# lasgroup/safe-adaptation-gym

Hardware: NVIDIA B200
Metric: env_steps_per_sec_point_go_to_goal (higher is better)
Workload: dtype f64

## Files before the change

include/sag_b200.h:

```cpp
#ifndef SAG_B200_H
#define SAG_B200_H
#include <stddef.h>
#include <stdint.h>

#ifdef __cplusplus
extern "C" {
#endif

#define SAG_ABI_VERSION 3
#define SAG_LIDAR_BINS 16
#define SAG_OBS_POINT 60
#define SAG_OBS_CAR 72
#define SAG_MAX_SLOTS 32
#define SAG_MAX_GREMLINS 4

enum { SAG_ROBOT_POINT = 0, SAG_ROBOT_CAR = 1 };
enum {
  SAG_T_CATCH_GOAL = 0, SAG_T_COLLECT, SAG_T_DRIBBLE_BALL, SAG_T_GO_TO_GOAL, SAG_T_GO_TO_GOAL_DAMPING,
  SAG_T_GO_TO_GOAL_MOTOR, SAG_T_GO_TO_GOAL_SCARCE, SAG_T_HAUL_BOX, SAG_T_PRESS_BUTTONS,
  SAG_T_PRESS_BUTTONS_SCARCE, SAG_T_PUSH_BOX, SAG_T_PUSH_BOX_SCARCE, SAG_T_ROLL_ROD, SAG_T_UNSUPERVISED,
  SAG_NUM_TASKS
};
enum { SAG_FLAG_PHYSICS_ERROR = 1, SAG_FLAG_RESAMPLE_FAILED = 2, SAG_FLAG_NEEDS_RESET = 4 };
enum { SAG_ERR_BAD_TASK_ID = 8 };

typedef struct SagConfig {
  int32_t n_envs;
  int32_t robot;
  uint64_t seed;
  uint32_t env_id_base;
  int32_t max_episode_steps;
  int32_t max_layout_draws;
  int32_t random_bound;
  double placements_margin, robot_keepout;
  double hazards_size, vases_size, pillars_size, gremlins_size;
  double hazards_keepout, gremlins_keepout, vases_keepout, pillars_keepout;
  double gremlins_travel, robot_ctrl_range_scale, action_noise, max_bound;
  int32_t num_gremlins;
  int32_t reserved_;
} SagConfig;

enum {
  SAG_F_ROBOT = 0,
  SAG_F_OBJECTS = 1,
  SAG_F_TASK_F64 = 2,
  SAG_F_TASK_I32 = 3,
  SAG_F_FLAGS = 4,
  SAG_F_ROBOT_EXT = 5,
  SAG_F_GREMLINS = 6,
  SAG_NUM_FIELDS
};

const char* sag_last_error(void);
int sag_abi_version(void);
void sag_default_config(SagConfig* cfg);

int sag_create(const SagConfig* cfg, int device, void** handle);
int sag_destroy(void* handle);
int sag_stride(void* handle);
int sag_obs_dim(void* handle);
size_t sag_field_bytes(void* handle, int field);
unsigned long long sag_launch_count(void* handle);
int sag_debug_read(void* handle, unsigned long long* out18_host);

int sag_set_tasks(void* handle, const int32_t* task_ids_dev, void* stream);
int sag_set_tasks_host(void* handle, const int32_t* task_ids_host);
int sag_bound_host(void* handle, double* bound_host);
int sag_error_flags(void* handle, int clear);

int sag_seed(void* handle, uint64_t seed);

int sag_reset(void* handle, const uint8_t* mask_dev, int only_flagged, int new_task, void* stream);
int sag_reset_obs(void* handle, const uint8_t* mask_dev, int only_flagged, int new_task, float* obs_dev, uint8_t* was_reset_dev,
                  void* stream);
int sag_reset_host(void* handle, const uint8_t* mask_host, int only_flagged, int new_task, float* obs_host);

int sag_step(void* handle, const float* act, float* obs, double* reward, double* reward2, uint8_t* cost, uint8_t* done,
// ... 28 lines not shown
```

safe_adaptation_gym_b200/_abi.py:

```python
import ctypes as C
import os

_HERE = os.path.dirname(os.path.abspath(__file__))
LIB_PATH = os.environ.get("SAG_B200_LIB") or os.path.join(_HERE, "csrc", "libsag_b200.so")

NUM_TASKS = 14
MAX_SLOTS = 32
MAX_GREMLINS = 4
F_ROBOT, F_OBJECTS, F_TASK_F64, F_TASK_I32, F_FLAGS, F_ROBOT_EXT, F_GREMLINS = range(7)
FLAG_PHYSICS_ERROR, FLAG_RESAMPLE_FAILED, FLAG_NEEDS_RESET, ERR_BAD_TASK_ID = 1, 2, 4, 8


class SagConfig(C.Structure):
    _fields_ = [
        ("n_envs", C.c_int32), ("robot", C.c_int32), ("seed", C.c_uint64), ("env_id_base", C.c_uint32),
        ("max_episode_steps", C.c_int32), ("max_layout_draws", C.c_int32), ("random_bound", C.c_int32),
        ("placements_margin", C.c_double), ("robot_keepout", C.c_double),
        ("hazards_size", C.c_double), ("vases_size", C.c_double), ("pillars_size", C.c_double), ("gremlins_size", C.c_double),
        ("hazards_keepout", C.c_double), ("gremlins_keepout", C.c_double), ("vases_keepout", C.c_double),
        ("pillars_keepout", C.c_double),
        ("gremlins_travel", C.c_double), ("robot_ctrl_range_scale", C.c_double), ("action_noise", C.c_double),
        ("max_bound", C.c_double),
        ("num_gremlins", C.c_int32), ("reserved_", C.c_int32),
    ]


class SagError(RuntimeError):
    pass


class SagLib:

    SYMBOLS = [
        "sag_last_error", "sag_abi_version", "sag_default_config", "sag_create", "sag_destroy", "sag_stride",
        "sag_obs_dim", "sag_field_bytes", "sag_launch_count", "sag_debug_read", "sag_set_tasks", "sag_set_tasks_host", "sag_bound_host",
        "sag_error_flags", "sag_reset_obs", "sag_reset_host", "sag_seed", "sag_reset", "sag_step", "sag_observe",
        "sag_step_host", "sag_observe_host", "sag_host_alloc", "sag_host_alloc_outputs", "sag_probe_d2h", "sag_host_free", "sag_rollout", "sag_read_field",
        "sag_write_field", "sag_task_stats", "sag_lidar", "sag_cost", "sag_export_outputs",
    ]

    def __init__(self, path, host_api=True):
        if not os.path.exists(path):
            raise SagError(
                f"{path} not found: build the CUDA extension first (python -c 'import __graft_entry__ as g; g.build()'). "
                "There is no CPU fallback.")
        self.path = path
        L = self.L = C.CDLL(path)
        vp, i32, u8p, fp, dp = C.c_void_p, C.c_int, C.c_void_p, C.c_void_p, C.c_void_p
        L.sag_last_error.restype = C.c_char_p
        L.sag_abi_version.restype = C.c_int
        L.sag_default_config.argtypes = [C.POINTER(SagConfig)]
        L.sag_create.argtypes = [C.POINTER(SagConfig), i32, C.POINTER(vp)]
        L.sag_destroy.argtypes = [vp]
        L.sag_stride.argtypes = [vp]
        L.sag_obs_dim.argtypes = [vp]
        L.sag_debug_read.argtypes = [vp, vp]
        L.sag_launch_count.restype = C.c_ulonglong
        L.sag_launch_count.argtypes = [vp]
        L.sag_field_bytes.restype = C.c_size_t
        L.sag_field_bytes.argtypes = [vp, i32]
        L.sag_set_tasks.argtypes = [vp, vp, vp]
        L.sag_seed.argtypes = [vp, C.c_uint64]
        L.sag_error_flags.argtypes = [vp, i32]
# ... 42 lines not shown
```

safe_adaptation_gym_b200/csrc/sag_core.cuh:

```cuda
#pragma once
#include <math.h>
#include <stdint.h>

#include "../../include/sag_detmath.h"

#if defined(__CUDACC__)
#define SAG_DEV_CONST __device__
#define SAG_HD __host__ __device__ __forceinline__
#define SAG_HD_NOINLINE __host__ __device__ __noinline__
#else
#define SAG_DEV_CONST
#define SAG_HD inline
#define SAG_HD_NOINLINE
#endif

#if defined(SAG_PROFILE) && !defined(__CUDACC__)
extern long* sag_prof_ptr;
#define SAG_PROF(e, i, n) do { if (sag_prof_ptr) sag_prof_ptr[(size_t)(e) * 16 + (i)] += (n); } while (0)
#define SAG_PROF_MAX(e, i, n) do { if (sag_prof_ptr && sag_prof_ptr[(size_t)(e) * 16 + (i)] < (n)) sag_prof_ptr[(size_t)(e) * 16 + (i)] = (n); } while (0)
#else
#define SAG_PROF(e, i, n) do { } while (0)
#define SAG_PROF_MAX(e, i, n) do { } while (0)
#endif

// ... 95 lines not shown

struct Dev;
SAG_HD TaskSpec spec_for(const Dev& D, int t, bool gremlins);

struct Slots {
  int h0, v0, g0, p0, t0, n;
  int goal, box, btn0, nbtn;
};
SAG_HD Slots make_slots(const TaskSpec& s) {
  Slots L;
  L.h0 = 0; L.v0 = s.nh; L.g0 = L.v0 + s.nv; L.p0 = L.g0 + s.ng; L.t0 = L.p0 + s.np;
  L.goal = L.box = L.btn0 = -1; L.nbtn = 0;
  if (s.kind == 0) { L.goal = L.t0; L.n = L.t0 + 1; }
  else if (s.kind == 1) { L.btn0 = L.t0; L.nbtn = s.nbuttons; L.n = L.t0 + s.nbuttons; }
  else { L.goal = L.t0; L.box = L.t0 + 1; L.n = L.t0 + 2; }
  return L;
}
SAG_HD int slot_kind(const TaskSpec& s, const Slots& L, int k) {
  if (k < L.v0) return K_HAZARD;
  if (k < L.g0) return K_VASE;
  if (k < L.p0) return K_GREMLIN;
  if (k < L.t0) return K_PILLAR;
  if (k == L.goal) return K_GOAL;
  if (k == L.box) return s.box_kind;
  return K_BUTTON;
}

struct Dev {
  int n, stride, nslots, robot;
  double action_noise, placements_margin, robot_keepout;
  double hazards_size, vases_size, pillars_size, gremlins_size;
  double k_hazard, k_vase, k_gremlin, k_pillar;
  double max_bound, ctrl_range_scale;
  int random_bound;
  unsigned long long seed;
  unsigned gid_base;
  int max_layout_draws, max_episode_steps;
  int num_gremlins;
  double gremlins_travel;
  double *rx, *ry, *ryaw, *rvx, *rvy, *rw;
  double *ctrl0, *ctrl1;
  double *cscale0, *cscale1, *bound;
  double* rext;
  double* grem;
  double *ox, *oy, *oyaw, *ovx, *ovy, *ow;
  int* task;
  double *last0, *last1;
  int *gbtn, *bstate, *btimer, *amask;
  double *cgcur, *cgnext, *cgox, *cgoy;
  int* cgtimer;
  int* movmask;
  int *worklist, *counts;
  int* counts_next;
  unsigned long long* dbg;
  int* errflags;
  double *time, *clear;
  unsigned *ctr, *episode;
  int* nstep;
  double *epret, *epcost;
  unsigned char* flags;
};

SAG_HD TaskSpec spec_for(const Dev& D, int t, bool gremlins) { TaskSpec s = task_spec(t); if (gremlins) s.ng = D.num_gremlins; return s; }
SAG_HD size_t oidx(const Dev& D, int slot, int e) { return (size_t)slot * D.stride + e; }

struct ObjView { double *x, *y, *yaw, *vx, *vy, *w; int stride; };
SAG_HD ObjView global_objects(const Dev& D, int e) {
  ObjView O = {D.ox + e, D.oy + e, D.oyaw + e, D.ovx + e, D.ovy + e, D.ow + e, D.stride};
  return O;
}

SAG_HD void philox4x32_10(uint32_t c0, uint32_t c1, uint32_t c2, uint32_t c3, uint32_t k0, uint32_t k1, uint32_t* out) {
#pragma unroll
  for (int r = 0; r < 10; ++r) {
    uint64_t p0 = (uint64_t)0xD2511F53u * c0, p1 = (uint64_t)0xCD9E8D57u * c2;
    uint32_t n0 = (uint32_t)(p1 >> 32) ^ c1 ^ k0, n1 = (uint32_t)p1;
    uint32_t n2 = (uint32_t)(p0 >> 32) ^ c3 ^ k1, n3 = (uint32_t)p0;
    c0 = n0; c1 = n1; c2 = n2; c3 = n3;
    k0 += 0x9E3779B9u; k1 += 0xBB67AE85u;
  }
  out[0] = c0; out[1] = c1; out[2] = c2; out[3] = c3;
}
struct Rng {
  uint64_t seed;
  uint32_t gid, episode;
  SAG_HD void pair(uint32_t stream, uint32_t ctr, double& u1, double& u2) const {
    uint32_t r[4];
    philox4x32_10(ctr, episode, gid, stream, (uint32_t)seed, (uint32_t)(seed >> 32), r);
    u1 = ((double)(r[0] >> 5) * 67108864.0 + (double)(r[1] >> 6)) * (1.0 / 9007199254740992.0);
    u2 = ((double)(r[2] >> 5) * 67108864.0 + (double)(r[3] >> 6)) * (1.0 / 9007199254740992.0);
  }
};

struct Geom { int is_box; double cx, cy, c, s, hx, hy, r; };
struct Hit { double nx, ny, px, py, dist; };

SAG_HD int hit_circle_circle(const Geom& A, const Geom& B, Hit* o) {
  double dx = B.cx - A.cx, dy = B.cy - A.cy;
  double len = sqrt(dx * dx + dy * dy);
  double dist = len - A.r - B.r;
  if (dist > 0.0) return 0;
  double nx = 1.0, ny = 0.0;
  if (len > 1e-14) { nx = dx / len; ny = dy / len; }
  o->nx = nx; o->ny = ny;
  o->px = A.cx + nx * (A.r + 0.5 * dist);
  o->py = A.cy + ny * (A.r + 0.5 * dist);
// ... 2379 lines not shown
```

safe_adaptation_gym_b200/csrc/sag_kernels.cu:

```cuda
#include <cuda_runtime.h>
#include <stdio.h>
#include <stdlib.h>
#include <string.h>
#include <time.h>

#include <new>

#include "../../include/sag_b200.h"
#include "sag_core.cuh"
#include "sag_layout.h"

using namespace sag;

namespace {

constexpr int kBS = 128;
constexpr int kTileStride = kBS + 1;
template <class RB>
struct TileCfg {
  static constexpr int kObs = RB::kObsDim;
  static constexpr size_t kTileBytes = (sizeof(float) * kObs * kTileStride + 15) / 16 * 16;
  static constexpr size_t kSmemBytes = kTileBytes + sizeof(Scratch) * (kBS / 32);
};

thread_local char g_err[512] = "";
void* g_packed_blocks[64];
bool is_packed_block(const void* p) {
  for (int k = 0; k < 64; ++k) if (g_packed_blocks[k] == p && p) return true;
  return false;
}

int fail(const char* what, cudaError_t ce = cudaSuccess) {
  if (ce != cudaSuccess) snprintf(g_err, sizeof(g_err), "%s: %s", what, cudaGetErrorString(ce));
  else snprintf(g_err, sizeof(g_err), "%s", what);
  return 1;
}
#define CK(call)                                   \
  do {                                             \
    cudaError_t ce_ = (call);                      \
    if (ce_ != cudaSuccess) return fail(#call, ce_); \
  } while (0)

struct DevGuard {
  int prev, want;
  explicit DevGuard(int d) : prev(-1), want(d) { if (cudaGetDevice(&prev) != cudaSuccess) prev = -1; if (prev != d) cudaSetDevice(d); }
  ~DevGuard() { if (prev >= 0 && prev != want) cudaSetDevice(prev); }
};

struct Handle {
  Dev D;
  int device;
  void* slab;
  size_t slab_bytes;
  void* field_ptr[SAG_NUM_FIELDS];
  size_t field_bytes[SAG_NUM_FIELDS];
  double *sret, *scost, *sn;
  double* stats_acc;
  int* err_h;
  int32_t* ids_d;
  uint8_t* mask_d;
  float* act_d;
  float* obs_d;
  double* rew_d;
  uint8_t *cost_d, *done_d;
  cudaStream_t own_stream;
  cudaStream_t copy_stream;
  cudaEvent_t ev_free, ev_copied;
  unsigned long long launches;
  int busy_grid;
};

template <int kObs>
__device__ __forceinline__ void write_tile(const float* tile, float* out, int e0, int n) {
  int cnt = min(kBS, n - e0) * kObs;
  float* dst = out + (size_t)e0 * kObs;
  for (int i = threadIdx.x; i < cnt; i += kBS) {
    int t = i / kObs, k = i - t * kObs;
    dst[i] = tile[k * kTileStride + t];
  }
}

template <int kObs>
__device__ __forceinline__ void write_tile4(const float* tile, float* out, int e0, int n) {
  static_assert(kObs % 4 == 0, "observation rows are written as float4");
  constexpr int kQ = kObs / 4;
  const int cnt = min(kBS, n - e0) * kQ;
  float4* dst = reinterpret_cast<float4*>(out + (size_t)e0 * kObs);
  for (int j = threadIdx.x; j < cnt; j += kBS) {
    const int t = j / kQ, q = j - t * kQ;
    const float* src = tile + (4 * q) * kTileStride + t;
    dst[j] = make_float4(src[0], src[kTileStride], src[2 * kTileStride], src[3 * kTileStride]);
  }
}

template <int kObs>
__device__ __forceinline__ void write_rows(const float* tile, int tstride, float* out, int e) {
  const int lane = threadIdx.x & 31;
#pragma unroll 4
  for (int r = 0; r < 32; ++r) {
    const int er = __shfl_sync(0xffffffffu, e, r);
    if (er < 0) continue;
    float* dst = out + (size_t)er * kObs;
    const float* src = tile + r;
    for (int k = lane; k < kObs; k += 32) dst[k] = src[k * tstride];
  }
}



template <class RB>
__global__ void __launch_bounds__(kBS, RB::kKind == 1 ? 2 : 4) k_step_free(Dev D, const float* __restrict__ act, float* __restrict__ obs,
                                                    double* __restrict__ reward, double* __restrict__ reward2,
                                                    uint8_t* __restrict__ cost, uint8_t* __restrict__ done) {
  constexpr int kObs = RB::kObsDim;
  extern __shared__ __align__(16) unsigned char smem_raw[];
  float* tile = reinterpret_cast<float*>(smem_raw);
  const int e = blockIdx.x * kBS + threadIdx.x;
  const int lane = threadIdx.x & 31;
  if (blockIdx.x == 0 && threadIdx.x < 4) D.counts_next[threadIdx.x] = 0;
  bool run = false, pretest = false;
  if (e < D.n) {
    RB R;
    load_robot(D, e, task_spec(D.task[e]), R);
    const unsigned char fl = D.flags[e];
    run = !(fl & F_PHYS_ERROR) && D.movmask[e] == 0 && D.num_gremlins == 0;
    pretest = !env_is_quiet(D.clear[e], R);
  }
  bool bail = false;
  if (run) {
    float2 a = reinterpret_cast<const float2*>(act)[e];
    double rew[2];
    unsigned char c, d;
    bail = env_step<kStepNear, RB>(0u, nullptr, D, e, a.x, a.y, tile + threadIdx.x, kTileStride, rew, &c, &d, pretest) != 0;
    if (!bail) {
      reward[e] = rew[0];
      if (reward2) { reward2[2 * e] = rew[0]; reward2[2 * e + 1] = rew[1]; }
      cost[e] = c;
      done[e] = d;
    }
  }
  const bool busy = e < D.n && (!run || bail);
  const unsigned m = __ballot_sync(0xffffffffu, busy);
  if (m) {
    int base = 0;
    if (lane == 0) base = atomicAdd(&D.counts[0], __popc(m));
    base = __shfl_sync(0xffffffffu, base, 0);
    if (busy) D.worklist[base + __popc(m & ((1u << lane) - 1u))] = e;
  }
  __syncthreads();
  write_tile4<kObs>(tile, obs, blockIdx.x * kBS, D.n);
}

constexpr int kCoopWarps = 16;
template <class RB>
struct CoopCfg {
  static constexpr int kObs = RB::kObsDim;
  static constexpr size_t kTileBytes = (sizeof(float) * kObs + 15) / 16 * 16;
  static constexpr size_t kPerWarp = kTileBytes + (sizeof(Scratch) + 15) / 16 * 16;
  static constexpr size_t kSmemBytes = kPerWarp * kCoopWarps;
};

template <class RB>
__global__ void __launch_bounds__(32 * kCoopWarps, 1) k_step_coop(const __grid_constant__ Dev D, const float* __restrict__ act,
                                                              float* __restrict__ obs, double* __restrict__ reward,
                                                              double* __restrict__ reward2, uint8_t* __restrict__ cost,
                                                              uint8_t* __restrict__ done) {
  extern __shared__ __align__(16) unsigned char smem_raw[];
  const int warp = threadIdx.x >> 5, lane = threadIdx.x & 31;
  unsigned char* mine = smem_raw + (size_t)warp * CoopCfg<RB>::kPerWarp;
  float* tile = reinterpret_cast<float*>(mine);
  Scratch* big = reinterpret_cast<Scratch*>(mine + CoopCfg<RB>::kTileBytes);
  cudaGridDependencySynchronize();
  const int count = D.counts[0];
  const int per_round = gridDim.x * kCoopWarps;
  for (int base = 0; base < count; base += per_round) {
    const int i = base + (warp * gridDim.x + blockIdx.x);
    if (i >= count) { coop_idle_step<RB>(); continue; }
    const int e = D.worklist[i];
#if defined(SAG_TIMING)
    if (lane == 0) { atomicAdd(&D.dbg[15], 1ull); big->tsum[0] = big->tsum[1] = big->tsum[2] = 0ull; }
    __syncwarp();
    long long clk_ = clock64();
#endif
    float2 a = reinterpret_cast<const float2*>(act)[e];
    double rew[2];
    unsigned char c, d;
    env_step<kStepCoop, RB>(0xffffffffu, big, D, e, a.x, a.y, tile, 1, rew, &c, &d);
#if defined(SAG_TIMING)
    if (lane == 0) {
      const unsigned long long tot = (unsigned long long)(clock64() - clk_);
      atomicAdd(&D.dbg[14], tot);
      const unsigned long long key = (tot << 40) | ((big->tsum[2] >> 10) << 20) | (big->tsum[0] >> 10);
      atomicMax(&D.dbg[16], key);
      atomicMax(&D.dbg[17], (tot << 40) | (big->tsum[1] >> 10));
    }
#endif
    __syncwarp();
    if (lane == 0) {
      reward[e] = rew[0];
      if (reward2) { reward2[2 * e] = rew[0]; reward2[2 * e + 1] = rew[1]; }
      cost[e] = c;
      done[e] = d;
    }
    float* dst = obs + (size_t)e * CoopCfg<RB>::kObs;
    for (int k = lane; k < CoopCfg<RB>::kObs; k += 32) dst[k] = tile[k];
    __syncwarp();
  }
}

template <class RB>
__global__ void __launch_bounds__(kBS) k_observe(Dev D, float* __restrict__ obs) {
  extern __shared__ __align__(16) unsigned char smem_raw[];
  float* tile = reinterpret_cast<float*>(smem_raw);
  Scratch* scratch = reinterpret_cast<Scratch*>(smem_raw + TileCfg<RB>::kTileBytes);
  const int e0 = blockIdx.x * kBS, e = e0 + threadIdx.x;
  const unsigned wmask = __ballot_sync(0xffffffffu, e < D.n);
  if (e < D.n) env_observe<RB>(wmask, &scratch[threadIdx.x >> 5], D, e, tile + threadIdx.x, kTileStride);
  __syncthreads();
  write_tile<RB::kObsDim>(tile, obs, e0, D.n);
}

__global__ void __launch_bounds__(256) k_rollout_actions(Dev D, float* __restrict__ act) {
  const int e = blockIdx.x * blockDim.x + threadIdx.x;
  if (e >= D.n) return;
  Rng rng = {D.seed, D.gid_base + (uint32_t)e, D.episode[e]};
  double u1, u2;
  rng.pair(2u, (uint32_t)D.nstep[e], u1, u2);
  reinterpret_cast<float2*>(act)[e] = make_float2((float)(2.0 * u1 - 1.0), (float)(2.0 * u2 - 1.0));
}

constexpr int kResetWarps = 4;
template <class RB>
struct ResetCfg {
  static constexpr size_t kRowBytes = (sizeof(float) * RB::kObsDim + 15) / 16 * 16;
  static constexpr size_t kPlaceBytes = 3 * 32 * sizeof(double);
  static constexpr size_t kPerWarp = kPlaceBytes + kRowBytes + (sizeof(Scratch) + 15) / 16 * 16;
  static constexpr size_t kSmemBytes = kPerWarp * kResetWarps;
};
template <class RB, bool WithObs>
__global__ void __launch_bounds__(32 * kResetWarps) k_reset(Dev D, const uint8_t* __restrict__ mask, int only_flagged, int new_task,
                                                            double* sret, double* scost, double* sn, float* __restrict__ obs,
                                                            uint8_t* __restrict__ was_reset, int gpc) {
  extern __shared__ __align__(16) unsigned char smem_raw[];
  const int warp = threadIdx.x >> 5, lane = threadIdx.x & 31;
  unsigned char* mine = smem_raw + (size_t)warp * (WithObs ? ResetCfg<RB>::kPerWarp : ResetCfg<RB>::kPlaceBytes);
  double* px = reinterpret_cast<double*>(mine);
  double* py = px + 32;
  double* pk = py + 32;
  float* row = reinterpret_cast<float*>(mine + ResetCfg<RB>::kPlaceBytes);
  Scratch* scratch = reinterpret_cast<Scratch*>(mine + ResetCfg<RB>::kPlaceBytes + ResetCfg<RB>::kRowBytes);
  const int e_l = blockIdx.x * gpc + lane;
  bool doit = lane < gpc && e_l < D.n;
  unsigned char fl_l = 0;
  if (doit) fl_l = D.flags[e_l];
  if (doit && mask && !mask[e_l]) doit = false;
  if (doit && only_flagged && !(fl_l & F_NEEDS_RESET)) doit = false;
  if (warp == 0 && lane < gpc && e_l < D.n && was_reset) was_reset[e_l] = doit ? 1 : 0;
  unsigned todo = __ballot_sync(0xffffffffu, doit);
  int rank = 0;
// ... 136 lines not shown
                                                    uint8_t* __restrict__ done_h) {
  const int lane = threadIdx.x & 31, nw = gridDim.x * 4;
  const int count = D.counts[0];
  for (int i = blockIdx.x * 4 + (threadIdx.x >> 5); i < count; i += nw) {
    const int e = D.worklist[i];
    const float* src = obs + (size_t)e * kObs;
    float* dst = obs_h + (size_t)e * kObs;
    for (int k = lane; k < kObs; k += 32) dst[k] = src[k];
    if (lane == 0) { reward_h[e] = reward[e]; cost_h[e] = cost[e]; done_h[e] = done[e]; }
  }
}

__global__ void __launch_bounds__(256) k_export_outputs(int n, int obs_quads, int reward_cols, const float4* __restrict__ obs,
                                                        const double* __restrict__ reward, const uint8_t* __restrict__ cost,
                                                        const uint8_t* __restrict__ done, const double* __restrict__ bound,
                                                        float4* __restrict__ obs_out, double* __restrict__ reward_out,
                                                        float* __restrict__ cost_out, uint8_t* __restrict__ done_out,
                                                        double* __restrict__ bound_out) {
  const size_t total = (size_t)n * obs_quads;
  for (size_t i = (size_t)blockIdx.x * blockDim.x + threadIdx.x; i < total; i += (size_t)gridDim.x * blockDim.x) {
    obs_out[i] = obs[i];
    if (i < (size_t)n) {
      for (int k = 0; k < reward_cols; ++k) reward_out[i * reward_cols + k] = reward[i * reward_cols + k];
      cost_out[i] = (float)cost[i];
      done_out[i] = done[i] ? 1 : 0;
      if (bound_out) bound_out[i] = bound[i];
    }
  }
}

static inline int grid_for(int n) { return (n + kBS - 1) / kBS; }

template <class RB>
struct Ops {
  static cudaError_t setup(Handle* H) {
    cudaError_t ce = cudaFuncSetAttribute(k_observe<RB>, cudaFuncAttributeMaxDynamicSharedMemorySize, (int)TileCfg<RB>::kSmemBytes);
    if (ce == cudaSuccess) ce = cudaFuncSetAttribute(k_reset<RB, true>, cudaFuncAttributeMaxDynamicSharedMemorySize, (int)ResetCfg<RB>::kSmemBytes);
    if (ce == cudaSuccess) ce = cudaFuncSetAttribute(k_step_coop<RB>, cudaFuncAttributeMaxDynamicSharedMemorySize, (int)CoopCfg<RB>::kSmemBytes);
    if (ce != cudaSuccess) return ce;
    {
      size_t need = 0;
      cudaFuncAttributes fa;
      if (cudaFuncGetAttributes(&fa, k_observe<RB>) == cudaSuccess && fa.localSizeBytes > need) need = fa.localSizeBytes;
      if (cudaFuncGetAttributes(&fa, k_reset<RB, true>) == cudaSuccess && fa.localSizeBytes > need) need = fa.localSizeBytes;
      need = (need + 255) / 256 * 256;
      size_t cur = 0;
      if (cudaDeviceGetLimit(&cur, cudaLimitStackSize) == cudaSuccess && cur < need) cudaDeviceSetLimit(cudaLimitStackSize, need);
      cudaGetLastError();
    }
    int sms = 148, per_sm = 1;
    cudaDeviceGetAttribute(&sms, cudaDevAttrMultiProcessorCount, H->device);
    ce = cudaOccupancyMaxActiveBlocksPerMultiprocessor(&per_sm, k_step_coop<RB>, 32 * kCoopWarps, CoopCfg<RB>::kSmemBytes);
    H->busy_grid = sms * (per_sm > 0 ? per_sm : 1);
    return ce;
  }
  static cudaError_t step(Handle* H, const float* act, float* obs, double* reward, double* reward2, uint8_t* cost, uint8_t* done,
                          cudaStream_t s) {
    cudaError_t ce = step_free(H, act, obs, reward, reward2, cost, done, s);
    if (ce != cudaSuccess) return ce;
    return step_coop(H, act, obs, reward, reward2, cost, done, s);
  }
  static cudaError_t step_free(Handle* H, const float* act, float* obs, double* reward, double* reward2, uint8_t* cost,
                               uint8_t* done, cudaStream_t s) {
    int* t = H->D.counts; H->D.counts = H->D.counts_next; H->D.counts_next = t;
    k_step_free<RB><<<grid_for(H->D.n), kBS, TileCfg<RB>::kTileBytes, s>>>(H->D, act, obs, reward, reward2, cost, done);
    ++H->launches;
    return cudaGetLastError();
  }
  static cudaError_t fixup_host(Handle* H, const float* obs, const double* reward, const uint8_t* cost, const uint8_t* done,
                                float* obs_h, double* reward_h, uint8_t* cost_h, uint8_t* done_h, cudaStream_t s) {
    k_fixup_host<RB::kObsDim><<<H->busy_grid, 128, 0, s>>>(H->D, obs, reward, cost, done, obs_h, reward_h, cost_h, done_h);
    ++H->launches;
    return cudaGetLastError();
  }
  static cudaError_t step_coop(Handle* H, const float* act, float* obs, double* reward, double* reward2, uint8_t* cost, uint8_t* done,
                               cudaStream_t s) {
    ++H->launches;
    const int need = (H->D.n + kCoopWarps - 1) / kCoopWarps;
    cudaLaunchConfig_t cfg = {};
    cfg.gridDim = dim3(need < H->busy_grid ? need : H->busy_grid);
    cfg.blockDim = dim3(32 * kCoopWarps);
    cfg.dynamicSmemBytes = CoopCfg<RB>::kSmemBytes;
    cfg.stream = s;
    cudaLaunchAttribute attr[1];
    attr[0].id = cudaLaunchAttributeProgrammaticStreamSerialization;
    attr[0].val.programmaticStreamSerializationAllowed = 1;
    cfg.attrs = attr;
    cfg.numAttrs = 1;
    return cudaLaunchKernelEx(&cfg, k_step_coop<RB>, H->D, act, obs, reward, reward2, cost, done);
  }
  static cudaError_t observe(Handle* H, float* obs, cudaStream_t s) {
    k_observe<RB><<<grid_for(H->D.n), kBS, TileCfg<RB>::kSmemBytes, s>>>(H->D, obs);
    ++H->launches;
    return cudaGetLastError();
  }
  static cudaError_t rollout(Handle* H, int k_steps, float* obs, double* reward, uint8_t* cost, uint8_t* done, cudaStream_t s) {
    float* o = obs ? obs : H->obs_d;
    double* r = reward ? reward : H->rew_d;
    uint8_t* c = cost ? cost : H->cost_d;
    uint8_t* d = done ? done : H->done_d;
    for (int k = 0; k < k_steps; ++k) {
      k_rollout_actions<<<(H->D.n + 255) / 256, 256, 0, s>>>(H->D, H->act_d);
      ++H->launches;
      cudaError_t ce = step(H, H->act_d, o, r, nullptr, c, d, s);
      if (ce != cudaSuccess) return ce;
    }
    return cudaGetLastError();
  }
  static cudaError_t reset(Handle* H, const uint8_t* mask, int only_flagged, int new_task, float* obs, uint8_t* was_reset, cudaStream_t s) {
    const int gpc = H->D.n <= 8192 ? kResetWarps : (H->D.n <= 16384 ? 2 * kResetWarps : (H->D.n <= 32768 ? 4 * kResetWarps : 32));
    const int grid = (H->D.n + gpc - 1) / gpc;
    ++H->launches;
    if (obs && (mask || only_flagged)) {
// ... 86 lines not shown
  CK(cudaDeviceSynchronize());
  CK(cudaMemcpy(out16, H->D.dbg, 18 * sizeof(unsigned long long), cudaMemcpyDeviceToHost));
  CK(cudaMemset(H->D.dbg, 0, 18 * sizeof(unsigned long long)));
  return 0;
}
unsigned long long sag_launch_count(void* handle) { return handle ? ((Handle*)handle)->launches : 0ull; }
int sag_stride(void* handle) { return ((Handle*)handle)->D.stride; }
int sag_obs_dim(void* handle) { return ((Handle*)handle)->D.robot == SAG_ROBOT_CAR ? SAG_OBS_CAR : SAG_OBS_POINT; }
size_t sag_field_bytes(void* handle, int field) {
  if (field < 0 || field >= SAG_NUM_FIELDS) return 0;
  return ((Handle*)handle)->field_bytes[field];
}

int sag_set_tasks(void* handle, const int32_t* ids, void* stream) {
  Handle* H = (Handle*)handle;
  if (!H || !ids) return fail("sag_set_tasks: null argument");
  DevGuard guard(H->device);
  k_set_tasks<<<(H->D.n + 255) / 256, 256, 0, (cudaStream_t)stream>>>(H->D, ids, H->sret, H->scost, H->sn, H->stats_acc);
  ++H->launches;
  CK(cudaGetLastError());
  return 0;
}

int sag_set_tasks_host(void* handle, const int32_t* ids_host) {
  Handle* H = (Handle*)handle;
  if (!H || !ids_host) return fail("sag_set_tasks_host: null argument");
  for (int e = 0; e < H->D.n; ++e)
    if (ids_host[e] < 0 || ids_host[e] >= SAG_NUM_TASKS) return fail("sag_set_tasks_host: task id out of range [0, SAG_NUM_TASKS)");
  DevGuard guard(H->device);
  CK(cudaDeviceSynchronize());
  CK(cudaMemcpyAsync(H->ids_d, ids_host, (size_t)H->D.n * sizeof(int32_t), cudaMemcpyHostToDevice, H->own_stream));
  k_set_tasks<<<(H->D.n + 255) / 256, 256, 0, H->own_stream>>>(H->D, H->ids_d, H->sret, H->scost, H->sn, H->stats_acc);
  ++H->launches;
  CK(cudaGetLastError());
  CK(cudaStreamSynchronize(H->own_stream));
  return 0;
}

int sag_bound_host(void* handle, double* bound_host) {
  Handle* H = (Handle*)handle;
  if (!H || !bound_host) return fail("sag_bound_host: null argument");
  DevGuard guard(H->device);
  CK(cudaDeviceSynchronize());
  CK(cudaMemcpy(bound_host, H->D.bound, (size_t)H->D.n * sizeof(double), cudaMemcpyDeviceToHost));
  return 0;
}

int sag_error_flags(void* handle, int clear) {
  Handle* H = (Handle*)handle;
  if (!H) return 0;
  int w = 0;
  if (H->err_h[0]) w |= SAG_FLAG_RESAMPLE_FAILED;
  if (H->err_h[1]) w |= SAG_ERR_BAD_TASK_ID;
  if (clear) { H->err_h[0] = 0; H->err_h[1] = 0; }
  return w;
}

int sag_seed(void* handle, uint64_t seed) {
  Handle* H = (Handle*)handle;
  if (!H) return fail("sag_seed: null handle");
  DevGuard guard(H->device);
  CK(cudaDeviceSynchronize());
  H->D.seed = seed;
  CK(cudaMemset(H->D.episode, 0xFF, (size_t)H->D.stride * sizeof(unsigned)));
  return 0;
}

int sag_reset(void* handle, const uint8_t* mask, int only_flagged, int new_task, void* stream) {
  Handle* H = (Handle*)handle;
  if (!H) return fail("sag_reset: null handle");
  DevGuard guard(H->device);
  CK(SAG_DISPATCH(H, reset(H, mask, only_flagged, new_task, nullptr, nullptr, (cudaStream_t)stream)));
  return 0;
}

int sag_reset_obs(void* handle, const uint8_t* mask, int only_flagged, int new_task, float* obs, uint8_t* was_reset, void* stream) {
  Handle* H = (Handle*)handle;
  if (!H || !obs) return fail("sag_reset_obs: null argument");
  DevGuard guard(H->device);
  CK(SAG_DISPATCH(H, reset(H, mask, only_flagged, new_task, obs, was_reset, (cudaStream_t)stream)));
  return 0;
}

int sag_reset_host(void* handle, const uint8_t* mask_h, int only_flagged, int new_task, float* obs_h) {
  Handle* H = (Handle*)handle;
  if (!H) return fail("sag_reset_host: null handle");
  DevGuard guard(H->device);
  cudaStream_t s = H->own_stream;
  CK(cudaDeviceSynchronize());
  const uint8_t* m = nullptr;
  if (mask_h) { CK(cudaMemcpyAsync(H->mask_d, mask_h, (size_t)H->D.n, cudaMemcpyHostToDevice, s)); m = H->mask_d; }
  CK(SAG_DISPATCH(H, reset(H, m, only_flagged, new_task, nullptr, nullptr, s)));
  if (obs_h) {
    CK(SAG_DISPATCH(H, observe(H, H->obs_d, s)));
    CK(cudaMemcpyAsync(obs_h, H->obs_d, (size_t)H->D.n * (size_t)sag_obs_dim(H) * sizeof(float), cudaMemcpyDeviceToHost, s));
  }
  CK(cudaStreamSynchronize(s));
  if (H->err_h[0]) return fail("sag_reset_host: failed to generate a layout (ResamplingError, world.py:189); see sag_error_flags");
  return 0;
}

int sag_step(void* handle, const float* act, float* obs, double* reward, double* reward2, uint8_t* cost, uint8_t* done,
             void* stream) {
  Handle* H = (Handle*)handle;
  if (!H || !act || !obs || !reward || !cost || !done) return fail("sag_step: null argument");
  DevGuard guard(H->device);
  CK(SAG_DISPATCH(H, step(H, act, obs, reward, reward2, cost, done, (cudaStream_t)stream)));
// ... 236 lines not shown
```

safe_adaptation_gym_b200/csrc/sag_layout.h:

```cpp
#pragma once
#include <stddef.h>
#include <stdint.h>
#include <string.h>

#include "../../include/sag_b200.h"
#include "sag_core.cuh"

namespace sag {

inline void default_config(SagConfig* c) {
  memset(c, 0, sizeof(*c));
  c->n_envs = 1; c->robot = SAG_ROBOT_POINT; c->seed = 666;
  c->placements_margin = 0.0; c->robot_keepout = 0.4;
  c->hazards_size = 0.2; c->vases_size = 0.1; c->pillars_size = 0.2; c->gremlins_size = 0.1;
  c->hazards_keepout = 0.18; c->gremlins_keepout = 0.4; c->vases_keepout = 0.15; c->pillars_keepout = 0.3;
  c->gremlins_travel = 0.35; c->robot_ctrl_range_scale = 0.0; c->action_noise = 0.01; c->max_bound = 25.0;
}

inline size_t align_up(size_t x, size_t a) { return (x + a - 1) / a * a; }

struct SlabLayout {
  size_t off[SAG_NUM_FIELDS], bytes[SAG_NUM_FIELDS];
  size_t stats_off, sched_off, act_off, obs_off, rew_off, cost_off, done_off, acc_off, ids_off, mask_off, total;
};

inline SlabLayout slab_layout(int n, int stride, int obs_dim) {
  SlabLayout L;
  const size_t st = (size_t)stride;
  L.bytes[SAG_F_ROBOT] = 6 * st * sizeof(double);
  L.bytes[SAG_F_OBJECTS] = 6 * (size_t)SAG_MAX_SLOTS * st * sizeof(double);
  L.bytes[SAG_F_TASK_F64] = 15 * st * sizeof(double);
  L.bytes[SAG_F_TASK_I32] = 10 * st * sizeof(int32_t);
  L.bytes[SAG_F_FLAGS] = st;
  L.bytes[SAG_F_ROBOT_EXT] = 6 * st * sizeof(double);
  L.bytes[SAG_F_GREMLINS] = (2 + 3 * (size_t)SAG_MAX_GREMLINS) * st * sizeof(double);
  size_t total = 0;
  for (int f = 0; f < SAG_NUM_FIELDS; ++f) { L.off[f] = total; total += align_up(L.bytes[f], 256); }
  L.stats_off = total; total += align_up(3 * st * sizeof(double), 256);
  L.sched_off = total; total += align_up((3 * st + 96) * sizeof(int32_t), 256);
  L.act_off = total; total += align_up((size_t)n * 2 * sizeof(float), 256);
  L.obs_off = total; total += align_up((size_t)n * obs_dim * sizeof(float), 256);
  L.rew_off = total; total += align_up((size_t)n * sizeof(double), 256);
  L.cost_off = total; total += align_up((size_t)n, 256);
  L.done_off = total; total += align_up((size_t)n, 256);
  L.acc_off = total; total += align_up(SAG_NUM_TASKS * 3 * sizeof(double), 256);
  L.ids_off = total; total += align_up((size_t)n * sizeof(int32_t), 256);
  L.mask_off = total; total += align_up((size_t)n, 256);
  L.total = total;
  return L;
}

inline void slab_bind(Dev& D, const SlabLayout& L, char* base) {
  const size_t st = (size_t)D.stride;
  double* r = (double*)(base + L.off[SAG_F_ROBOT]);
  D.rx = r; D.ry = r + st; D.ryaw = r + 2 * st; D.rvx = r + 3 * st; D.rvy = r + 4 * st; D.rw = r + 5 * st;
  double* o = (double*)(base + L.off[SAG_F_OBJECTS]);
  const size_t os = (size_t)SAG_MAX_SLOTS * st;
  D.ox = o; D.oy = o + os; D.oyaw = o + 2 * os; D.ovx = o + 3 * os; D.ovy = o + 4 * os; D.ow = o + 5 * os;
  double* t = (double*)(base + L.off[SAG_F_TASK_F64]);
  D.last0 = t; D.last1 = t + st; D.cgcur = t + 2 * st; D.cgnext = t + 3 * st; D.cgox = t + 4 * st; D.cgoy = t + 5 * st;
  D.time = t + 6 * st; D.clear = t + 7 * st; D.epret = t + 8 * st; D.epcost = t + 9 * st; D.ctrl0 = t + 10 * st; D.ctrl1 = t + 11 * st;
  D.cscale0 = t + 12 * st; D.cscale1 = t + 13 * st; D.bound = t + 14 * st;
  int32_t* ii = (int32_t*)(base + L.off[SAG_F_TASK_I32]);
  D.task = ii; D.gbtn = ii + st; D.bstate = ii + 2 * st; D.btimer = ii + 3 * st; D.amask = ii + 4 * st; D.cgtimer = ii + 5 * st;
  D.nstep = ii + 6 * st; D.ctr = (unsigned*)(ii + 7 * st); D.episode = (unsigned*)(ii + 8 * st); D.movmask = ii + 9 * st;
  D.flags = (unsigned char*)(base + L.off[SAG_F_FLAGS]);
  D.rext = (double*)(base + L.off[SAG_F_ROBOT_EXT]);
  D.grem = (double*)(base + L.off[SAG_F_GREMLINS]);
  int32_t* sc = (int32_t*)(base + L.sched_off);
  D.worklist = sc; D.counts = sc + 3 * st; D.counts_next = D.counts + 8;
  D.dbg = (unsigned long long*)(sc + 3 * st + 16);
}

inline void dev_from_config(Dev& D, const SagConfig& c) {
  D.n = c.n_envs;
  D.stride = (int)align_up((size_t)c.n_envs, 32);
  D.nslots = SAG_MAX_SLOTS;
  D.robot = c.robot;
  D.action_noise = c.action_noise; D.placements_margin = c.placements_margin; D.robot_keepout = c.robot_keepout;
  D.hazards_size = c.hazards_size; D.vases_size = c.vases_size; D.pillars_size = c.pillars_size; D.gremlins_size = c.gremlins_size;
  D.k_hazard = c.hazards_keepout < c.hazards_size ? c.hazards_size : c.hazards_keepout;
  D.k_vase = c.vases_keepout < c.vases_size ? c.vases_size : c.vases_keepout;
  D.k_gremlin = c.gremlins_keepout < c.gremlins_size ? c.gremlins_size : c.gremlins_keepout;
  D.k_pillar = c.pillars_keepout < c.pillars_size ? c.pillars_size : c.pillars_keepout;
  D.max_bound = c.max_bound; D.ctrl_range_scale = c.robot_ctrl_range_scale; D.random_bound = c.random_bound;
  D.seed = c.seed; D.gid_base = c.env_id_base;
  D.max_layout_draws = c.max_layout_draws; D.max_episode_steps = c.max_episode_steps;
  D.num_gremlins = c.num_gremlins; D.gremlins_travel = c.gremlins_travel;
}

}
```

safe_adaptation_gym_b200/env.py:

```python
import ctypes as C
from typing import Dict, Optional, Sequence, Union

import numpy as np
import torch

from safe_adaptation_gym_b200 import _abi
from safe_adaptation_gym_b200 import tasks as _tasks
from safe_adaptation_gym_b200.spaces import Box
from safe_adaptation_gym_b200.utils import ResamplingError

WORLD_DEFAULT = {
    'placements_margin': 0.0, 'robot_keepout': 0.4, 'hazards_size': 0.2, 'vases_size': 0.1, 'pillars_size': 0.2,
    'gremlins_size': 0.1, 'hazards_keepout': 0.18, 'gremlins_keepout': 0.4, 'vases_keepout': 0.15,
    'pillars_keepout': 0.3, 'gremlins_travel': 0.35, 'obstacles_size_noise_scale': 0.0,
    'robot_ctrl_range_scale': 0.0, 'action_noise': 0.01, 'max_bound': 25, 'random_bound': False,
}
_EXTRA_KEYS = {'max_layout_draws', 'num_gremlins'}
_ROBOT_TO_CONTROL_FREQUENCY = {'doggo': 12, 'point': 5, 'car': 10}


def _robot_name(path: str) -> str:
    base = path.replace('\\', '/').split('/')[-1]
    return base[:-4] if base.endswith('.xml') else base

# ... 57 lines not shown
            setattr(c, k, float(cfg[k]))
        self._seed = int(np.random.randint(2**32))
        c.seed = self._seed
        self._h = C.c_void_p()
        L.check(L.L.sag_create(C.byref(c), dev_index, C.byref(self._h)))
        self.stride = L.L.sag_stride(self._h)
        self.obs_dim = L.L.sag_obs_dim(self._h)
        self.max_episode_steps = int(max_episode_steps)
        self.env_id_base = int(env_id_base)
        self.copy_outputs = bool(copy_outputs)
        n, dev = self.num_envs, self.device
        self._obs = torch.empty((n, self.obs_dim), dtype=torch.float32, device=dev)
        self._reward = torch.empty((n,), dtype=torch.float64, device=dev)
        self._reward2 = torch.empty((n, 2), dtype=torch.float64, device=dev)
        self._cost = torch.empty((n,), dtype=torch.uint8, device=dev)
        self._done = torch.empty((n,), dtype=torch.uint8, device=dev)
        self._was_reset = torch.zeros((n,), dtype=torch.uint8, device=dev)
        self._bound = torch.full((n,), float(cfg['max_bound']), dtype=torch.float64, device=dev)
        self._task_ids = None
        self._tasks = None
        self._any_unsupervised = False
        self._action_space = Box(-1, 1, (2,), dtype=np.float32)
        self._observation_space = None

    def __del__(self):
        try:
            if getattr(self, '_h', None):
                self._lib.L.sag_destroy(self._h)
                self._h = None
        except Exception:
            pass

    def close(self):
        self.__del__()

    def _stream(self):
        if self.device.type == 'cuda':
            return C.c_void_p(torch.cuda.current_stream(self.device).cuda_stream)
        return C.c_void_p(0)

    @staticmethod
    def _p(t):
        return C.c_void_p(t.data_ptr()) if t is not None else None

    def _out(self, t):
        return t.clone() if self.copy_outputs else t

    def _raise_recorded_errors(self, where: str):
        w = self._lib.L.sag_error_flags(self._h, 1)
        if w & _abi.FLAG_RESAMPLE_FAILED:
            raise ResamplingError('Failed to generate goal' if where == 'step' else 'Failed to generate layout')
        if w & _abi.ERR_BAD_TASK_ID:
            raise ValueError('task id out of range')

    def step(self, action):
        act = self._as_action(action)
        L = self._lib
        r2 = self._reward2 if self._any_unsupervised else None
        L.check(L.L.sag_step(self._h, self._p(act), self._p(self._obs), self._p(self._reward), self._p(r2),
                             self._p(self._cost), self._p(self._done), self._stream()))
        reward = self._reward2 if self._any_unsupervised else self._reward
        was_reset = None
        if self.max_episode_steps > 0:
            L.check(L.L.sag_reset_obs(self._h, None, 1, 0, self._p(self._obs), self._p(self._was_reset), self._stream()))
            was_reset = self._was_reset.to(torch.bool)
        if self.copy_outputs:
            n, dev = self.num_envs, self.device
            obs = torch.empty((n, self.obs_dim), dtype=torch.float32, device=dev)
            rew = torch.empty_like(reward)
            cost = torch.empty((n,), dtype=torch.float32, device=dev)
            done = torch.empty((n,), dtype=torch.bool, device=dev)
            bound = torch.empty((n,), dtype=torch.float64, device=dev)
            L.check(L.L.sag_export_outputs(self._h, self._p(self._obs), self._p(reward), 2 if self._any_unsupervised else 1,
                                           self._p(self._cost), self._p(self._done), self._p(self._bound), self._p(obs), self._p(rew),
                                           self._p(cost), self._p(done), self._p(bound), self._stream()))
        else:
            obs, rew, bound = self._obs, reward, self._bound
            cost, done = self._cost.to(torch.float32), self._done.view(torch.bool)
        info = {'cost': cost, 'bound': bound}
        if was_reset is not None:
            info['truncated'] = was_reset & ~done
            done = done | was_reset
        self._raise_recorded_errors('step')
        return obs, rew, done, info

    def reset(self, *, seed: Optional[int] = None, return_info: bool = False, options: Optional[dict] = None):
        assert self._task_ids is not None or (options is not None and 'task' in options), (
            'A task should be first set before reset.')
        if seed is not None:
            self.seed(seed)
        if options is not None and 'task' in options:
            self.set_task(options['task'])
            return self.observation
        self._reset_all(new_task=False)
        return self.observation

    def seed(self, seed=None):
        self._seed = int(np.random.randint(2**32)) if seed is None else int(seed)
        self._lib.check(self._lib.L.sag_seed(self._h, C.c_uint64(self._seed)))

    def set_task(self, task):
        if isinstance(task, _tasks.Task):
            task_list = [task] * self.num_envs
        else:
            task_list = list(task)
            if len(task_list) != self.num_envs:
# ... 125 lines not shown
```

Before: 246.1 million.

## Fuse batch and cooperative step kernels into one persistent cooperative launch

For non-car robots, the separate k_step_free and k_step_coop launches are replaced by one cooperative kernel. Blocks first run the fast batch path over slices and publish busy environments into a generation-tagged global queue with release stores. Then every block pulls queued environments for warp-cooperative stepping while slices are still finishing. This removes a kernel launch and the serialisation between the two phases, and lets the slow path overlap with the batch path. In exchange it adds spin-waits with acquire loads, atomics and a timeout error flag, which could hurt when the queue is usually empty.

Measured after the change: 253.4 million, median of 6. 1.03x the previous value.

```diff
diff --git a/include/sag_b200.h b/include/sag_b200.h
--- a/include/sag_b200.h
+++ b/include/sag_b200.h
@@ -22,7 +22,7 @@
   SAG_NUM_TASKS
 };
 enum { SAG_FLAG_PHYSICS_ERROR = 1, SAG_FLAG_RESAMPLE_FAILED = 2, SAG_FLAG_NEEDS_RESET = 4 };
-enum { SAG_ERR_BAD_TASK_ID = 8 };
+enum { SAG_ERR_BAD_TASK_ID = 8, SAG_ERR_STEP_STALLED = 16 };
 
 typedef struct SagConfig {
   int32_t n_envs;
diff --git a/safe_adaptation_gym_b200/_abi.py b/safe_adaptation_gym_b200/_abi.py
--- a/safe_adaptation_gym_b200/_abi.py
+++ b/safe_adaptation_gym_b200/_abi.py
@@ -8,7 +8,7 @@
 MAX_SLOTS = 32
 MAX_GREMLINS = 4
 F_ROBOT, F_OBJECTS, F_TASK_F64, F_TASK_I32, F_FLAGS, F_ROBOT_EXT, F_GREMLINS = range(7)
-FLAG_PHYSICS_ERROR, FLAG_RESAMPLE_FAILED, FLAG_NEEDS_RESET, ERR_BAD_TASK_ID = 1, 2, 4, 8
+FLAG_PHYSICS_ERROR, FLAG_RESAMPLE_FAILED, FLAG_NEEDS_RESET, ERR_BAD_TASK_ID, ERR_STEP_STALLED = 1, 2, 4, 8, 16
 
 
 class SagConfig(C.Structure):
diff --git a/safe_adaptation_gym_b200/csrc/sag_core.cuh b/safe_adaptation_gym_b200/csrc/sag_core.cuh
--- a/safe_adaptation_gym_b200/csrc/sag_core.cuh
+++ b/safe_adaptation_gym_b200/csrc/sag_core.cuh
@@ -171,6 +171,8 @@
   int* movmask;
   int *worklist, *counts;
   int* counts_next;
+  unsigned long long* queue;
+  unsigned gen;
   unsigned long long* dbg;
   int* errflags;
   double *time, *clear;
diff --git a/safe_adaptation_gym_b200/csrc/sag_kernels.cu b/safe_adaptation_gym_b200/csrc/sag_kernels.cu
--- a/safe_adaptation_gym_b200/csrc/sag_kernels.cu
+++ b/safe_adaptation_gym_b200/csrc/sag_kernels.cu
@@ -68,6 +68,7 @@
   cudaEvent_t ev_free, ev_copied;
   unsigned long long launches;
   int busy_grid;
+  int step_grid;
 };
 
 template <int kObs>
@@ -81,13 +82,14 @@
 }
 
 template <int kObs>
-__device__ __forceinline__ void write_tile4(const float* tile, float* out, int e0, int n) {
+__device__ __forceinline__ void write_tile4(const float* tile, float* out, int e0, int n, int tid, const unsigned* skip) {
   static_assert(kObs % 4 == 0, "observation rows are written as float4");
   constexpr int kQ = kObs / 4;
   const int cnt = min(kBS, n - e0) * kQ;
   float4* dst = reinterpret_cast<float4*>(out + (size_t)e0 * kObs);
-  for (int j = threadIdx.x; j < cnt; j += kBS) {
+  for (int j = tid; j < cnt; j += kBS) {
     const int t = j / kQ, q = j - t * kQ;
+    if (skip && (skip[t >> 5] >> (t & 31) & 1u)) continue;
     const float* src = tile + (4 * q) * kTileStride + t;
     dst[j] = make_float4(src[0], src[kTileStride], src[2 * kTileStride], src[3 * kTileStride]);
   }
@@ -107,6 +109,30 @@
 }
 
 
+
+template <class RB>
+__device__ __forceinline__ bool batch_decide(const Dev& D, int e, bool& pretest) {
+  RB R;
+  load_robot(D, e, task_spec(D.task[e]), R);
+  const unsigned char fl = D.flags[e];
+  const bool run = !(fl & F_PHYS_ERROR) && D.movmask[e] == 0 && D.num_gremlins == 0;
+  pretest = !env_is_quiet(D.clear[e], R);
+  return run;
+}
+template <class RB>
+__device__ __forceinline__ bool batch_step(const Dev& D, int e, bool pretest, const float* __restrict__ act, float* col,
+                                           double* __restrict__ reward, double* __restrict__ reward2, uint8_t* __restrict__ cost,
+                                           uint8_t* __restrict__ done) {
+  float2 a = reinterpret_cast<const float2*>(act)[e];
+  double rew[2];
+  unsigned char c, d;
+  if (env_step<kStepNear, RB>(0u, nullptr, D, e, a.x, a.y, col, kTileStride, rew, &c, &d, pretest) != 0) return true;
+  reward[e] = rew[0];
+  if (reward2) { reward2[2 * e] = rew[0]; reward2[2 * e + 1] = rew[1]; }
+  cost[e] = c;
+  done[e] = d;
+  return false;
+}
 
 template <class RB>
 __global__ void __launch_bounds__(kBS, RB::kKind == 1 ? 2 : 4) k_step_free(Dev D, const float* __restrict__ act, float* __restrict__ obs,
@@ -119,26 +145,9 @@
   const int lane = threadIdx.x & 31;
   if (blockIdx.x == 0 && threadIdx.x < 4) D.counts_next[threadIdx.x] = 0;
   bool run = false, pretest = false;
-  if (e < D.n) {
-    RB R;
-    load_robot(D, e, task_spec(D.task[e]), R);
-    const unsigned char fl = D.flags[e];
-    run = !(fl & F_PHYS_ERROR) && D.movmask[e] == 0 && D.num_gremlins == 0;
-    pretest = !env_is_quiet(D.clear[e], R);
-  }
+  if (e < D.n) run = batch_decide<RB>(D, e, pretest);
   bool bail = false;
-  if (run) {
-    float2 a = reinterpret_cast<const float2*>(act)[e];
-    double rew[2];
-    unsigned char c, d;
-    bail = env_step<kStepNear, RB>(0u, nullptr, D, e, a.x, a.y, tile + threadIdx.x, kTileStride, rew, &c, &d, pretest) != 0;
-    if (!bail) {
-      reward[e] = rew[0];
-      if (reward2) { reward2[2 * e] = rew[0]; reward2[2 * e + 1] = rew[1]; }
-      cost[e] = c;
-      done[e] = d;
-    }
-  }
+  if (run) bail = batch_step<RB>(D, e, pretest, act, tile + threadIdx.x, reward, reward2, cost, done);
   const bool busy = e < D.n && (!run || bail);
   const unsigned m = __ballot_sync(0xffffffffu, busy);
   if (m) {
@@ -148,7 +157,7 @@
     if (busy) D.worklist[base + __popc(m & ((1u << lane) - 1u))] = e;
   }
   __syncthreads();
-  write_tile4<kObs>(tile, obs, blockIdx.x * kBS, D.n);
+  write_tile4<kObs>(tile, obs, blockIdx.x * kBS, D.n, threadIdx.x, nullptr);
 }
 
 constexpr int kCoopWarps = 16;
@@ -161,12 +170,48 @@
 };
 
 template <class RB>
+__device__ __forceinline__ void coop_env(const Dev& D, int e, Scratch* big, float* tile, const float* __restrict__ act,
+                                         float* __restrict__ obs, double* __restrict__ reward, double* __restrict__ reward2,
+                                         uint8_t* __restrict__ cost, uint8_t* __restrict__ done) {
+  const int lane = threadIdx.x & 31;
+#if defined(SAG_TIMING)
+  const unsigned long long known_ = (D.movmask[e] != 0 || (D.flags[e] & F_PHYS_ERROR)) ? 1ull : 0ull;
+  if (lane == 0) { atomicAdd(&D.dbg[15], 1ull + (known_ << 32)); big->tsum[0] = big->tsum[1] = big->tsum[2] = 0ull; }
+  __syncwarp();
+  long long clk_ = clock64();
+#endif
+  float2 a = reinterpret_cast<const float2*>(act)[e];
+  double rew[2];
+  unsigned char c, d;
+  env_step<kStepCoop, RB>(0xffffffffu, big, D, e, a.x, a.y, tile, 1, rew, &c, &d);
+#if defined(SAG_TIMING)
+  if (lane == 0) {
+    const unsigned long long tot = (unsigned long long)(clock64() - clk_);
+    atomicAdd(&D.dbg[14], tot);
+    const unsigned long long key = (tot << 40) | (known_ << 39) | (((big->tsum[2] >> 10) & 0x7ffffull) << 20) | (big->tsum[0] >> 10);
+    atomicMax(&D.dbg[16], key);
+    atomicMax(&D.dbg[17], (tot << 40) | (big->tsum[1] >> 10));
+  }
+#endif
+  __syncwarp();
+  if (lane == 0) {
+    reward[e] = rew[0];
+    if (reward2) { reward2[2 * e] = rew[0]; reward2[2 * e + 1] = rew[1]; }
+    cost[e] = c;
+    done[e] = d;
+  }
+  float* dst = obs + (size_t)e * CoopCfg<RB>::kObs;
+  for (int k = lane; k < CoopCfg<RB>::kObs; k += 32) dst[k] = tile[k];
+  __syncwarp();
+}
+
+template <class RB>
 __global__ void __launch_bounds__(32 * kCoopWarps, 1) k_step_coop(const __grid_constant__ Dev D, const float* __restrict__ act,
                                                               float* __restrict__ obs, double* __restrict__ reward,
                                                               double* __restrict__ reward2, uint8_t* __restrict__ cost,
                                                               uint8_t* __restrict__ done) {
   extern __shared__ __align__(16) unsigned char smem_raw[];
-  const int warp = threadIdx.x >> 5, lane = threadIdx.x & 31;
+  const int warp = threadIdx.x >> 5;
   unsigned char* mine = smem_raw + (size_t)warp * CoopCfg<RB>::kPerWarp;
   float* tile = reinterpret_cast<float*>(mine);
   Scratch* big = reinterpret_cast<Scratch*>(mine + CoopCfg<RB>::kTileBytes);
@@ -176,35 +221,129 @@
   for (int base = 0; base < count; base += per_round) {
     const int i = base + (warp * gridDim.x + blockIdx.x);
     if (i >= count) { coop_idle_step<RB>(); continue; }
-    const int e = D.worklist[i];
-#if defined(SAG_TIMING)
-    if (lane == 0) { atomicAdd(&D.dbg[15], 1ull); big->tsum[0] = big->tsum[1] = big->tsum[2] = 0ull; }
-    __syncwarp();
-    long long clk_ = clock64();
-#endif
-    float2 a = reinterpret_cast<const float2*>(act)[e];
-    double rew[2];
-    unsigned char c, d;
-    env_step<kStepCoop, RB>(0xffffffffu, big, D, e, a.x, a.y, tile, 1, rew, &c, &d);
-#if defined(SAG_TIMING)
-    if (lane == 0) {
-      const unsigned long long tot = (unsigned long long)(clock64() - clk_);
-      atomicAdd(&D.dbg[14], tot);
-      const unsigned long long key = (tot << 40) | ((big->tsum[2] >> 10) << 20) | (big->tsum[0] >> 10);
-      atomicMax(&D.dbg[16], key);
-      atomicMax(&D.dbg[17], (tot << 40) | (big->tsum[1] >> 10));
-    }
-#endif
-    __syncwarp();
-    if (lane == 0) {
-      reward[e] = rew[0];
-      if (reward2) { reward2[2 * e] = rew[0]; reward2[2 * e + 1] = rew[1]; }
-      cost[e] = c;
-      done[e] = d;
-    }
-    float* dst = obs + (size_t)e * CoopCfg<RB>::kObs;
-    for (int k = lane; k < CoopCfg<RB>::kObs; k += 32) dst[k] = tile[k];
-    __syncwarp();
+    coop_env<RB>(D, D.worklist[i], big, tile, act, obs, reward, reward2, cost, done);
+  }
+}
+
+constexpr int kSlice = 32 * kCoopWarps;
+constexpr unsigned long long kWaitNs = 1000000000ull;
+
+__device__ __forceinline__ unsigned long long global_ns() {
+  unsigned long long t;
+  asm volatile("mov.u64 %0, %%globaltimer;" : "=l"(t));
+  return t;
+}
+__device__ __forceinline__ int ld_acquire(const int* p) {
+  int v;
+  asm volatile("ld.acquire.gpu.global.b32 %0, [%1];" : "=r"(v) : "l"(p) : "memory");
+  return v;
+}
+__device__ __forceinline__ unsigned long long ld_acquire(const unsigned long long* p) {
+  unsigned long long v;
+  asm volatile("ld.acquire.gpu.global.b64 %0, [%1];" : "=l"(v) : "l"(p) : "memory");
+  return v;
+}
+__device__ __forceinline__ void st_release(unsigned long long* p, unsigned long long v) {
+  asm volatile("st.release.gpu.global.b64 [%0], %1;" ::"l"(p), "l"(v) : "memory");
+}
+
+__device__ __forceinline__ unsigned publish(const Dev& D, bool pub, int e) {
+  const int lane = threadIdx.x & 31;
+  const unsigned m = __ballot_sync(0xffffffffu, pub);
+  if (m) {
+    int base = 0;
+    if (lane == 0) base = atomicAdd(&D.counts[0], __popc(m));
+    base = __shfl_sync(0xffffffffu, base, 0);
+    if (pub) st_release(&D.queue[base + __popc(m & ((1u << lane) - 1u))], ((unsigned long long)D.gen << 32) | (unsigned)e);
+  }
+  return m;
+}
+
+template <class RB>
+struct StepCfg {
+  static constexpr size_t kBatchBytes = (kSlice / kBS) * TileCfg<RB>::kTileBytes;
+  static constexpr size_t kSmemBytes = kBatchBytes > CoopCfg<RB>::kSmemBytes ? kBatchBytes : CoopCfg<RB>::kSmemBytes;
+};
+
+template <class RB>
+__global__ void __launch_bounds__(kSlice, 1) k_step(const __grid_constant__ Dev D, const float* __restrict__ act,
+                                                   float* __restrict__ obs, double* __restrict__ reward,
+                                                   double* __restrict__ reward2, uint8_t* __restrict__ cost,
+                                                   uint8_t* __restrict__ done) {
+  constexpr int kObs = RB::kObsDim;
+  extern __shared__ __align__(16) unsigned char smem_raw[];
+  __shared__ unsigned handed[kCoopWarps];
+  __shared__ int round_first, round_take;
+  const int warp = threadIdx.x >> 5, lane = threadIdx.x & 31;
+  const int slices = (D.n + kSlice - 1) / kSlice;
+  if (blockIdx.x == 0 && threadIdx.x < 4) D.counts_next[threadIdx.x] = 0;
+
+  for (int sl = blockIdx.x; sl < slices; sl += gridDim.x) {
+    const int e = sl * kSlice + threadIdx.x;
+    const int q = threadIdx.x / kBS, t = threadIdx.x & (kBS - 1);
+    float* tile = reinterpret_cast<float*>(smem_raw + q * TileCfg<RB>::kTileBytes);
+    bool run = false, pretest = false;
+    if (e < D.n) run = batch_decide<RB>(D, e, pretest);
+    unsigned m = publish(D, e < D.n && !run, e);
+    if (lane == 0) { __threadfence(); atomicAdd(&D.counts[3], 1); }
+    bool bail = false;
+    if (run) bail = batch_step<RB>(D, e, pretest, act, tile + t, reward, reward2, cost, done);
+    m |= publish(D, bail, e);
+    if (lane == 0) handed[warp] = m;
+    __syncthreads();
+    if (threadIdx.x == 0) { __threadfence(); atomicAdd(&D.counts[2], 1); }
+    write_tile4<kObs>(tile, obs, sl * kSlice + q * kBS, D.n, t, handed + q * (kBS / 32));
+    __syncthreads();
+  }
+
+  unsigned char* mine = smem_raw + (size_t)warp * CoopCfg<RB>::kPerWarp;
+  float* tile = reinterpret_cast<float*>(mine);
+  Scratch* big = reinterpret_cast<Scratch*>(mine + CoopCfg<RB>::kTileBytes);
+  bool first_round = true;
+  for (;;) {
+    if (threadIdx.x == 0) {
+      const unsigned long long deadline = global_ns() + kWaitNs;
+      unsigned ns = 32;
+      if (first_round && blockIdx.x >= slices)
+        while (ld_acquire(&D.counts[3]) < slices * kCoopWarps) {
+          if (global_ns() > deadline) { D.errflags[2] = 1; break; }
+          __nanosleep(ns); ns = ns < 1024 ? 2 * ns : ns;
+        }
+      int f = 0, k = -1;
+      for (;;) {
+        const int sdone = ld_acquire(&D.counts[2]);
+        const int r = ld_acquire(&D.counts[0]);
+        f = *(volatile int*)&D.counts[1];
+        if (r > f) {
+          const int want = min(kCoopWarps, r - f);
+          if (atomicCAS(&D.counts[1], f, f + want) == f) { k = want; break; }
+          continue;
+        }
+        if (sdone == slices) break;
+        if (global_ns() > deadline) { D.errflags[2] = 1; break; }
+        __nanosleep(ns); ns = ns < 1024 ? 2 * ns : ns;
+      }
+      round_first = f; round_take = k;
+    }
+    __syncthreads();
+    const int f = round_first, k = round_take;
+    first_round = false;
+    if (k < 0) break;
+    int e = -1;
+    if (warp < k) {
+      if (lane == 0) {
+        const unsigned long long deadline = global_ns() + kWaitNs;
+        unsigned long long v;
+        while (((v = ld_acquire(&D.queue[f + warp])) >> 32) != D.gen) {
+          if (global_ns() > deadline) { D.errflags[2] = 1; break; }
+          __nanosleep(32);
+        }
+        if ((v >> 32) == D.gen) e = (int)(unsigned)v;
+      }
+      e = __shfl_sync(0xffffffffu, e, 0);
+    }
+    if (e >= 0) coop_env<RB>(D, e, big, tile, act, obs, reward, reward2, cost, done);
+    else coop_idle_step<RB>();
   }
 }
 
@@ -447,13 +586,43 @@
     cudaDeviceGetAttribute(&sms, cudaDevAttrMultiProcessorCount, H->device);
     ce = cudaOccupancyMaxActiveBlocksPerMultiprocessor(&per_sm, k_step_coop<RB>, 32 * kCoopWarps, CoopCfg<RB>::kSmemBytes);
     H->busy_grid = sms * (per_sm > 0 ? per_sm : 1);
+    if (ce != cudaSuccess) return ce;
+    if constexpr (kFused) {
+      int coop = 0;
+      ce = cudaDeviceGetAttribute(&coop, cudaDevAttrCooperativeLaunch, H->device);
+      if (ce == cudaSuccess && !coop) ce = cudaErrorNotSupported;
+      if (ce == cudaSuccess) ce = cudaFuncSetAttribute(k_step<RB>, cudaFuncAttributeMaxDynamicSharedMemorySize, (int)StepCfg<RB>::kSmemBytes);
+      if (ce == cudaSuccess) ce = cudaOccupancyMaxActiveBlocksPerMultiprocessor(&per_sm, k_step<RB>, kSlice, StepCfg<RB>::kSmemBytes);
+      if (ce == cudaSuccess && per_sm < 1) ce = cudaErrorInvalidConfiguration;
+      H->step_grid = sms * per_sm;
+    }
     return ce;
   }
+  static constexpr bool kFused = RB::kKind != 1;
   static cudaError_t step(Handle* H, const float* act, float* obs, double* reward, double* reward2, uint8_t* cost, uint8_t* done,
                           cudaStream_t s) {
-    cudaError_t ce = step_free(H, act, obs, reward, reward2, cost, done, s);
-    if (ce != cudaSuccess) return ce;
-    return step_coop(H, act, obs, reward, reward2, cost, done, s);
+    if constexpr (kFused) {
+      int* t = H->D.counts; H->D.counts = H->D.counts_next; H->D.counts_next = t;
+      if (++H->D.gen == 0u) ++H->D.gen;
+      const int slices = (H->D.n + kSlice - 1) / kSlice, need = (H->D.n + kCoopWarps - 1) / kCoopWarps;
+      const int want = slices > need ? slices : need;
+      cudaLaunchConfig_t cfg = {};
+      cfg.gridDim = dim3(want < H->step_grid ? want : H->step_grid);
+      cfg.blockDim = dim3(kSlice);
+      cfg.dynamicSmemBytes = StepCfg<RB>::kSmemBytes;
+      cfg.stream = s;
+      cudaLaunchAttribute attr[1];
+      attr[0].id = cudaLaunchAttributeCooperative;
+      attr[0].val.cooperative = 1;
+      cfg.attrs = attr;
+      cfg.numAttrs = 1;
+      ++H->launches;
+      return cudaLaunchKernelEx(&cfg, k_step<RB>, H->D, act, obs, reward, reward2, cost, done);
+    } else {
+      cudaError_t ce = step_free(H, act, obs, reward, reward2, cost, done, s);
+      if (ce != cudaSuccess) return ce;
+      return step_coop(H, act, obs, reward, reward2, cost, done, s);
+    }
   }
   static cudaError_t step_free(Handle* H, const float* act, float* obs, double* reward, double* reward2, uint8_t* cost,
                                uint8_t* done, cudaStream_t s) {
@@ -646,7 +815,8 @@
   int w = 0;
   if (H->err_h[0]) w |= SAG_FLAG_RESAMPLE_FAILED;
   if (H->err_h[1]) w |= SAG_ERR_BAD_TASK_ID;
-  if (clear) { H->err_h[0] = 0; H->err_h[1] = 0; }
+  if (H->err_h[2]) w |= SAG_ERR_STEP_STALLED;
+  if (clear) { H->err_h[0] = 0; H->err_h[1] = 0; H->err_h[2] = 0; }
   return w;
 }
 
diff --git a/safe_adaptation_gym_b200/csrc/sag_layout.h b/safe_adaptation_gym_b200/csrc/sag_layout.h
--- a/safe_adaptation_gym_b200/csrc/sag_layout.h
+++ b/safe_adaptation_gym_b200/csrc/sag_layout.h
@@ -69,6 +69,7 @@
   D.grem = (double*)(base + L.off[SAG_F_GREMLINS]);
   int32_t* sc = (int32_t*)(base + L.sched_off);
   D.worklist = sc; D.counts = sc + 3 * st; D.counts_next = D.counts + 8;
+  D.queue = (unsigned long long*)(sc + st);
   D.dbg = (unsigned long long*)(sc + 3 * st + 16);
 }
 
diff --git a/safe_adaptation_gym_b200/env.py b/safe_adaptation_gym_b200/env.py
--- a/safe_adaptation_gym_b200/env.py
+++ b/safe_adaptation_gym_b200/env.py
@@ -133,6 +133,8 @@
             raise ResamplingError('Failed to generate goal' if where == 'step' else 'Failed to generate layout')
         if w & _abi.ERR_BAD_TASK_ID:
             raise ValueError('task id out of range')
+        if w & _abi.ERR_STEP_STALLED:
+            raise RuntimeError('a wait inside the step kernel passed its deadline: the results of that step are incomplete')
 
     def step(self, action):
         act = self._as_action(action)
```
